# pettni/smooth_feedback

Hardware: AMD Instinct MI355X
Metric: QP solves/sec (higher is better)
Workload: dtype f64

## Files before the change

smooth_feedback_amd/csrc/qp_sparse.hip:

```cpp
#include <hip/hip_runtime.h>

#include <cstdlib>
#include <map>
#include <mutex>

#include <algorithm>
#include <type_traits>
#include <utility>
#include <cfloat>
#include <cmath>

#include "knobs.h"
#include "../../include/sfb.h"
#include "qp_sparse_kernel.h"
#include "wave_util.h"

#ifndef SFB_SWEEP_ASM
#define SFB_SWEEP_ASM 1
#endif
#ifndef SFB_SWEEP_DEPTH
#define SFB_SWEEP_DEPTH 8
#endif

namespace sfb {

namespace {

__device__ __forceinline__ int uni(const int v) { return __builtin_amdgcn_readfirstlane(v); }

struct Ws {
  double *Lx, *LxF, *LxB, *D, *Dinv, *tv;
  double *sx, *qc, *xs, *xus, *dxus;
  double *sy, *rho, *rinv, *lo, *hi, *ys, *zs, *yus, *zus, *dyus, *act;
  double *hdr;
  double *Axc;
};
constexpr int kHdrStamp = 6, kHdrC = 7, kHdrSigma = 8, kHdrScaling = 9;
constexpr int kHdrCode = 10, kHdrComplete = 11;
[[maybe_unused]] constexpr int kHdrTl2 = 12;
enum { PH_SETUP = 1, PH_ADMM = 2, PH_FINISH = 3 };
constexpr int phases_pack(int ph0, int ph1, unsigned pause_at = 0, int dq_mode = 0)
{
  return ph0 | (ph1 << 4) | (int)((pause_at & 0xFFFFFu) << 8) | (dq_mode << 28);
}
constexpr int PH_EVERYTHING = phases_pack(PH_SETUP, PH_FINISH);
constexpr unsigned long long kFactorStamp = 0x5FB0FAC7A11CE5EDull;

__device__ __forceinline__ Ws carve_ws(double *base, int n, int m, int nnzL, int funits, int bunits)
{
  const int k = n + m;
  Ws w;
  double *p = base;
  w.Lx = p; p += nnzL;
  w.D = p; p += k;
  p += 2;
  w.LxF = p; p += (size_t)(funits + kSweepPadDev) * 128;
  w.LxB = p; p += (size_t)(bunits + kSweepPadDev) * 128;
  w.Dinv = p; p += k;   w.tv = p; p += k;
  w.sx = p; p += n;     w.qc = p; p += n;     w.xs = p; p += n;   w.xus = p; p += n;  w.dxus = p; p += n;
  p += n;
  w.sy = p; p += m;     w.rho = p; p += m;    w.rinv = p; p += m; w.lo = p; p += m;   w.hi = p; p += m;
  w.ys = p; p += m;     w.zs = p; p += m;     w.yus = p; p += m;  w.zus = p; p += m;  w.dyus = p; p += m;
  w.act = p; p += m;
  w.hdr = p; p += 16;
  w.Axc = p;
  return w;
}
__device__ __forceinline__ Ws polish_ws(const Ws &w, double *base, const size_t off, int n, int m, int nnzL, int funits, int bunits)
{
  const int k = n + m;
  Ws v = w;
  double *p = base + off;
  v.Lx = p; p += nnzL;
  v.D = p; p += k;
  p += 2;
  v.LxF = p; p += (size_t)(funits + kSweepPadDev) * 128;
  v.LxB = p; p += (size_t)(bunits + kSweepPadDev) * 128;
  v.Dinv = p;
// ... 847 lines not shown
__device__ inline void ldl_solve_dev(const SparsePlanDev &pl, const Ws &w, double *t, const int lane, const bool lean,
                                     const double *dinv_lds = nullptr)
{
  const double *const Dinv = dinv_lds ? dinv_lds : w.Dinv;
  const int k = uni(pl.k);
  const bool bo = uni(pl.idx_scale) == 8;
  auto sweep = [&](const int32_t *idx, const int units, const double *vals, const int32_t *mask, const int f0, const int f1) {
    if (lean) {
      vdouble2 lx[SFB_SWEEP_DEPTH];
      vint2 ix[SFB_SWEEP_DEPTH];
      if (bo) sweep_dev<SFB_SWEEP_DEPTH, true, true>(idx, units, vals, t, lane, mask, f0, f1, lx, ix);
      else sweep_dev<SFB_SWEEP_DEPTH, false, true>(idx, units, vals, t, lane, mask, f0, f1, lx, ix);
    } else {
      vdouble2 lx[SD];
      vint2 ix[SD];
      if (bo) sweep_dev<SD, true, false>(idx, units, vals, t, lane, mask, f0, f1, lx, ix);
      else sweep_dev<SD, false, false>(idx, units, vals, t, lane, mask, f0, f1, lx, ix);
    }
  };
  sweep(pl.fidx, uni(pl.funits), w.LxF, pl.fmask, uni(pl.ffull0), uni(pl.ffull1));
  for (int j0 = lane; j0 < k; j0 += kWave * 8) {
    double dv[8];
#pragma unroll
    for (int e = 0; e < 8; ++e) dv[e] = (j0 + e * kWave < k) ? Dinv[j0 + e * kWave] : 0.0;
#pragma unroll
    for (int e = 0; e < 8; ++e)
      if (j0 + e * kWave < k) t[j0 + e * kWave] = dv[e] * t[j0 + e * kWave];
  }
  wave_sync();
  sweep(pl.bidx, uni(pl.bunits), w.LxB, pl.bmask, uni(pl.bfull0), uni(pl.bfull1));
}

constexpr int kLatRegRows = 12;
__host__ __device__ constexpr size_t lat_lds_doubles(const int n, const int m)
{
  const size_t lay = (size_t)(((n + m + 2) + 1) & ~1) + n + 2 * (size_t)m + (n + m) + 8 + (2 * kLatRegRows * 64) / 4 + (kLatRegRows * 64) / 8 + 4;
  const size_t rows = (size_t)(((n + m + 2) + 1) & ~1) + kLatRegRows * 64;
  return lay > rows ? lay : rows;
}
#ifndef SFB_LAT_TAIL
#define SFB_LAT_TAIL 48
#endif
constexpr int kLatTail = SFB_LAT_TAIL;
constexpr int kLatTailMax = 48;
static_assert(kLatTail >= 0 && kLatTail <= kLatTailMax && kLatTail % 8 == 0, "the forward sweep ends on a block of 8 units; lanes 0 .. kLatTail");
constexpr int kLatTailReg0 = 256 - 2 * kLatTail;
constexpr int kLatResident = ((kLatTailReg0 - kAgprFree) / 4) & ~7;
__device__ __forceinline__ int lat_tail_units(const SparsePlanDev &pl)
{
  const int ft = uni(pl.ftail);
  return (kLatTail > 0 && uni(pl.idx_scale) == 8 && uni(pl.ftail0) >= 8) ? (ft < kLatTail ? ft : kLatTail) : 0;
}
__device__ __forceinline__ bool lat_resident_ok(const SparsePlanDev &pl, const int treg) { return uni(pl.funits) - treg >= kLatResident + 16; }
__device__ __forceinline__ void lat_resident_load(const double *LxF, const int lane)
{
  asm volatile("" ::: "a255");
  const vdouble2 *p = reinterpret_cast<const vdouble2 *>(LxF) + lane;
  auto for_units = [&]<int... U>(std::integer_sequence<int, U...>, auto &&fn) { (fn(std::integral_constant<int, U>{}), ...); };
  for_units(std::make_integer_sequence<int, kLatResident / 4>{}, [&]<int G>(std::integral_constant<int, G>) {
    const vdouble2 *pg = p + G * 4 * kWave;
    asm volatile("global_load_dwordx4 a[%1:%2], %0, off\n\t"
                 "global_load_dwordx4 a[%3:%4], %0, off offset:1024\n\t"
                 "global_load_dwordx4 a[%5:%6], %0, off offset:2048\n\t"
                 "global_load_dwordx4 a[%7:%8], %0, off offset:3072"
                 :
                 : "v"(pg), "n"(kAgprFree + 16 * G), "n"(kAgprFree + 16 * G + 3), "n"(kAgprFree + 16 * G + 4), "n"(kAgprFree + 16 * G + 7),
                   "n"(kAgprFree + 16 * G + 8), "n"(kAgprFree + 16 * G + 11), "n"(kAgprFree + 16 * G + 12), "n"(kAgprFree + 16 * G + 15)
                 : "memory");
  });
  asm volatile("s_waitcnt vmcnt(0)" ::: "memory");
}
__device__ __forceinline__ unsigned long long lat_tail_load(const SparsePlanDev &pl, const double *LxF, const int lane, const int treg)
{
  asm volatile("" ::: "a255");
  unsigned long long have = 0;
  const int i0 = uni(pl.ftail) - kLatTail;
  const int32_t *pos = pl.ftpos + (lane + i0);
  auto for_steps = [&]<int... S>(std::integer_sequence<int, S...>, auto &&fn) { (fn(std::integral_constant<int, S>{}), ...); };
  for_steps(std::make_integer_sequence<int, kLatTail>{}, [&]<int S>(std::integral_constant<int, S>) {
    const bool on = S >= kLatTail - treg && lane > S && lane <= kLatTail;
    const int q   = on ? pos[(i0 + S) * kWave] : -1;
    const double *pv = LxF + (q >= 0 ? q : 0);
    asm volatile("global_load_dwordx2 a[%1:%2], %0, off" : : "v"(pv), "n"(kLatTailReg0 + 2 * S), "n"(kLatTailReg0 + 2 * S + 1) : "memory");
    if (q >= 0) have |= 1ull << S;
  });
  asm volatile("s_waitcnt vmcnt(0)" ::: "memory");
  return have;
}
__device__ __forceinline__ void ldl_solve_lat(const SparsePlanDev &pl, const Ws &w, double *t, const int lane, const double *Dinv,
                                              vdouble2 (&lx)[8], vint2 (&ix)[8], const bool pre, const bool next, const bool resident = false,
                                              const int treg = 0, const unsigned long long tail_have = 0)
{
  const int k = uni(pl.k);
  const int fu = uni(pl.funits) - treg;
  if (resident) sweep_dev<8, true, false, false, true, kLatResident>(pl.fidx, fu, w.LxF, t, lane, pl.fmask, 0, 0, lx, ix, pl.bidx, w.LxB, pl.bmask);
  else if (pre) sweep_dev<8, true, false, true, true>(pl.fidx, fu, w.LxF, t, lane, pl.fmask, 0, 0, lx, ix, pl.bidx, w.LxB, pl.bmask);
  else sweep_dev<8, true, false, false, true>(pl.fidx, fu, w.LxF, t, lane, pl.fmask, 0, 0, lx, ix, pl.bidx, w.LxB, pl.bmask);
  if constexpr (kLatTail > 0) {
    if (treg > 0) {
      double *const tl = t + (k - 1 - kLatTail) + lane;
      const bool mine = lane >= kLatTail - treg && lane <= kLatTail;
      double tr = mine ? *tl : 0.0;
      auto for_steps = [&]<int... S>(std::integer_sequence<int, S...>, auto &&fn) { (fn(std::integral_constant<int, S>{}), ...); };
      auto block = [&]<int B>(std::integral_constant<int, B>) {
        if (8 * B + 8 > kLatTail - treg) {
          for_steps(std::make_integer_sequence<int, 8>{}, [&]<int E>(std::integral_constant<int, E>) {
            constexpr int S = 8 * B + E;
            int l0, h0;
            asm volatile("v_accvgpr_read_b32 %0, a[%2] ; lat tail (check_sweep_spills.py)\n\tv_accvgpr_read_b32 %1, a[%3]"
                         : "=v"(l0), "=v"(h0)
                         : "n"(kLatTailReg0 + 2 * S), "n"(kLatTailReg0 + 2 * S + 1));
            const double piv = __hiloint2double(__builtin_amdgcn_readlane(__double2hiint(tr), S), __builtin_amdgcn_readlane(__double2loint(tr), S));
            if ((tail_have >> S) & 1) tr = fma(-__hiloint2double(h0, l0), piv, tr);
          });
        }
      };
      for_steps(std::make_integer_sequence<int, kLatTail / 8>{}, block);
      if (mine && lane > kLatTail - treg) *tl = tr;
      wave_lds_fence();
    }
  }
  for (int j0 = lane; j0 < k; j0 += kWave * 8) {
    double dv[8];
#pragma unroll
    for (int e = 0; e < 8; ++e) dv[e] = (j0 + e * kWave < k) ? Dinv[j0 + e * kWave] : 0.0;
#pragma unroll
    for (int e = 0; e < 8; ++e)
      if (j0 + e * kWave < k) t[j0 + e * kWave] = dv[e] * t[j0 + e * kWave];
  }
  wave_lds_fence();
  if (next) sweep_dev<8, true, false, true, true>(pl.bidx, uni(pl.bunits), w.LxB, t, lane, pl.bmask, 0, 0, lx, ix, pl.fidx, w.LxF, pl.fmask);
  else sweep_dev<8, true, false, true, false>(pl.bidx, uni(pl.bunits), w.LxB, t, lane, pl.bmask, 0, 0, lx, ix);
}

template<int UB>
__device__ __forceinline__ double lane_max_abs_b(const double *v, const int len, const int lane)
{
  double r = 0.0;
  for (int e0 = lane; e0 < len; e0 += kWave * UB) {
    double x[UB];
#pragma unroll
    for (int e = 0; e < UB; ++e) x[e] = (e0 + e * kWave < len) ? v[e0 + e * kWave] : 0.0;
#pragma unroll
    for (int e = 0; e < UB; ++e) r = fmax(r, fabs(x[e]));
  }
  return wave_max(r);
}
__device__ __forceinline__ double lane_max_abs(const double *v, int len, int lane)
{
  double r = 0.0;
// ... 691 lines not shown
      for (int e = 0; e < UB; ++e)
        if (p0 + e * kWave < nnzA) w.Axc[p0 + e * kWave] = v[e];
    }
    it.Ax = w.Axc;
    wave_sync();
  }

  bool keep_scaling = keep && !kp.scaling;
  if (kp.scaling) {
    for (int j = lane; j < n; j += kWave) {
      double v = 0.0;
      for (int p = pl.Pp[j]; p < pl.Pp[j + 1]; ++p) v = fmax(v, fabs(it.Px[p]));
      if (v == 0.0) v = 1.0;
      t[j] = v;
    }
    wave_sync();
    double sum = t[0];
    {
      int j = 1;
      for (; j + 16 <= n; j += 16) {
        double v[16];
#pragma unroll
        for (int qq = 0; qq < 16; ++qq) v[qq] = t[j + qq];
#pragma unroll
        for (int qq = 0; qq < 16; ++qq) sum += v[qq];
      }
      for (; j < n; ++j) sum += t[j];
    }
    const double qn = lane_max_abs(it.q, n, lane);
    c               = 1.0 / fmax(fmax(1e-6, sum / (double)n), qn);
    wave_sync();
    keep_scaling = keep && c == w.hdr[kHdrC];
  }
  if (!keep_scaling) {
    for (int j = lane; j < n; j += kWave) w.sx[j] = 1.0;
    for (int i = lane; i < m; i += kWave) w.sy[i] = 1.0;
    wave_sync();
  }
  if (kp.scaling && !keep_scaling) {
    int pass = 0;
    double crit;
    do {
      for (int e = lane; e < k; e += kWave) t[e] = 0.0;
      wave_sync();
      constexpr int UB = 8;
      {
        int rr[UB], cc[UB];
        double pv[UB];
        auto fetchP = [&](const int p0) {
#pragma unroll
          for (int e = 0; e < UB; ++e) {
            const int p = p0 + e * kWave;
            const bool on = p < nnzP;
            rr[e] = on ? pl.Pi[p] : 0;
            cc[e] = on ? pl.Pcol[p] : 0;
            pv[e] = on ? it.Px[p] : 0.0;
          }
        };
        fetchP(lane);
        for (int p0 = lane; p0 < nnzP; p0 += kWave * UB) {
          int c0[UB];
          double v0[UB], sr[UB], sc[UB];
#pragma unroll
          for (int e = 0; e < UB; ++e) {
            sr[e] = w.sx[rr[e]];
            sc[e] = w.sx[cc[e]];
            c0[e] = cc[e];
            v0[e] = pv[e];
          }
          fetchP(p0 + kWave * UB);
#pragma unroll
          for (int e = 0; e < UB; ++e)
// ... 26 lines not shown
            c0[e] = cc[e];
            v0[e] = av[e];
          }
          fetchA(p0 + kWave * UB);
#pragma unroll
          for (int e = 0; e < UB; ++e) {
            if (p0 + e * kWave < nnzA) {
              const double v = fabs(sr[e] * sc[e] * v0[e]);
              __hip_atomic_fetch_max(&t[c0[e]], v, __ATOMIC_RELAXED, __HIP_MEMORY_SCOPE_WORKGROUP);
              __hip_atomic_fetch_max(&t[n + r0[e]], v, __ATOMIC_RELAXED, __HIP_MEMORY_SCOPE_WORKGROUP);
            }
          }
        }
      }
      wave_sync();
      double cm = 0.0;
      for (int e = lane; e < k; e += kWave) {
        double inc = t[e];
        if (inc == 0.0) inc = 1.0;
        t[e] = inc;
        cm   = fmax(cm, fabs(inc - 1.0));
      }
      wave_sync();
      for (int j = lane; j < n; j += kWave) w.sx[j] = sqrt(1.0 / fmax(t[j], 1e-8)) * w.sx[j];
      for (int i = lane; i < m; i += kWave) w.sy[i] = sqrt(1.0 / fmax(t[n + i], 1e-8)) * w.sy[i];
      crit = wave_max(cm);
      wave_sync();
    } while (pass++ < 10 && crit > 0.1);
  }

  bool keep_factor = keep_scaling;
  {
    bool bad = false, rho_changed = false;
    for (int i = lane; i < m; i += kWave) {
      const double li = it.l[i], ui = it.u[i], syi = w.sy[i];
      bad = bad || (li == inf) || (ui == -inf) || (ui - li < 0.0);
      double rho;
      if (li == -inf && ui == inf) rho = 1e-6;
      else if (syi * fabs(li - ui) < 1e-5) rho = 1e3 * kp.rho_bar;
      else rho = kp.rho_bar;
      if (keep_scaling) rho_changed = rho_changed || !(w.rho[i] == rho);
      w.rho[i]  = rho;
      w.rinv[i] = 1.0 / rho;
      w.lo[i]   = syi * li;
      w.hi[i]   = syi * ui;
    }
    for (int j = lane; j < n; j += kWave) w.qc[j] = c * w.sx[j] * it.q[j];
    if (wave_ballot(bad)) ret_code = SFB_QP_PRIMAL_INFEASIBLE;
    if (keep_scaling && wave_ballot(rho_changed)) keep_factor = false;
  }
  wave_sync();

  phase_lap(0);
  if (!keep_factor) {
    if (lane == 0) w.hdr[kHdrStamp] = 0.0;
    if (!ldl_numeric_dev<8>(pl, it, w, t, 0, c, kp.sigma, kp.delta, lane, TRACE ? &ph_fill : nullptr)) {
      ret_code = SFB_QP_UNKNOWN;
    } else if (lane == 0 && allow_reuse) {
      w.hdr[kHdrStamp]   = __longlong_as_double((long long)kFactorStamp);
      w.hdr[kHdrC]       = c;
      w.hdr[kHdrSigma]   = kp.sigma;
      w.hdr[kHdrScaling] = (double)kp.scaling;
    }
  }

  if constexpr (TRACE) {
    phase_lap(2);
    ph_t[1] = ph_fill;
    ph_t[2] -= ph_fill;
  }
#ifdef SFB_SP_TIMELINE
  tl1 = wall_clock64();
#endif
  if (gwx != nullptr) {
    const double *wx = gwx + b * (size_t)n, *wy = gwy + b * (size_t)m;
    for (int j = lane; j < n; j += kWave) w.xs[j] = (1.0 / w.sx[j]) * wx[j];
    for (int i = lane; i < m; i += kWave) {
      const double syi = w.sy[i];
      w.ys[i]          = c * ((1.0 / syi) * wy[i]);
      double acc       = 0.0;
// ... 704 lines not shown
      }
    }
    item   = __builtin_amdgcn_readfirstlane(item);
    resume = __builtin_amdgcn_readfirstlane(resume);
    const int lean_waves_item = lean_waves;
    if (item < 0) break;
    if (resume) __builtin_amdgcn_fence(__ATOMIC_ACQUIRE, "agent");
    const bool helper = LAT && resume == 2;
    if (dq_mode == 2 || helper) resume = 0;
    wave_sync();
    const SparsePlanDev *use = plp;
    double *wsb              = gws;
    size_t wsd = ws_doubles, slot = (queue == nullptr) ? (size_t)blockIdx.x : (size_t)item;
    int fbslot = -1;
    if (plf != nullptr && !resume && ph0 <= PH_SETUP && !sp_guard_ok(*plp, gAx + (size_t)item * (size_t)uni(plp->nnzA_io), lane)) {
      if (lane == 0) {
        for (int probe = blockIdx.x % nfb;; probe = (probe + 1) % nfb) {
          if (atomicCAS(&fbflags[probe], 0, 1) == 0) { fbslot = probe; break; }
          __builtin_amdgcn_s_sleep(8);
        }
      }
      fbslot = __builtin_amdgcn_readfirstlane(fbslot);
      use = plf; wsb = gwsf; wsd = wsf_doubles; slot = (size_t)fbslot;
    }
    int seen = 0;
    const bool counts_own = dq_mode == 2 || (LAT && ((phases >> 28) & 1) == 1);
    if (counts_own && lane == 0) atomicAdd(&(fbflags + kFbSlots + 2 * batch + 16)[kDqOwn], 1);
    int32_t *const active = plp->dev_active;
    if (lane == 0) seen = atomicAdd(active, 1);
    const bool lean = (nwaves > lean_waves_item) || __builtin_amdgcn_readfirstlane(seen) >= lean_waves_item;
    const int st = sp_solve_item<LAT, TRACE, LAT || POLISHER>(*use, kp, gPx, gq, gAx, gl, gu, gwx, gwy, gx, gy, gobj, giter, gcode, wsb, wsd, lean_waves_item,
                                 lean, (size_t)item, slot, t, lane, resume != 0, fbslot >= 0 ? nullptr : queue, nfresh, slice,
                                  fbslot < 0 && slot == (size_t)item,
                                 fbslot >= 0 ? PH_EVERYTHING : (helper ? (PH_FINISH | (PH_FINISH << 4)) : phases), keys ? keys + item : nullptr, trace,
                                 trace_cap, phase_us);
    if (keys != nullptr && st != SP_PAUSED && lane == 0) keys[item] = -1.0f;
    if (fbslot >= 0 && phases != PH_EVERYTHING && lane == 0)
      carve_ws(gws + (size_t)item * ws_doubles, uni(plp->n), uni(plp->m), uni(plp->nnzL), uni(plp->funits), uni(plp->bunits)).hdr[kHdrComplete] = 1.0;
    if ((dq_mode == 2 || helper) && lane == 0)
      carve_ws(gws + (size_t)item * ws_doubles, uni(plp->n), uni(plp->m), uni(plp->nnzL), uni(plp->funits), uni(plp->bunits)).hdr[kHdrComplete] = 1.0;
    wave_sync();
    if constexpr (LAT) {
      if (st == SP_DONE && !helper && (phases & 0xFF) == (PH_ADMM | (PH_ADMM << 4)) && ((phases >> 28) & 1) == 1 && lane == 0) {
        int32_t *const doneq = fbflags + kFbSlots + 2 * batch + 16;
        __builtin_amdgcn_fence(__ATOMIC_RELEASE, "agent");
        asm volatile("s_waitcnt vmcnt(0)" ::: "memory");
        const int tl = atomicAdd(&doneq[kDqTail], 1);
        __hip_atomic_store(&doneq[kDqRing + tl], item + 1, __ATOMIC_RELAXED, __HIP_MEMORY_SCOPE_AGENT);
      }
    }
    if (lane == 0) {
      atomicSub(active, 1);
      if (counts_own) atomicSub(&(fbflags + kFbSlots + 2 * batch + 16)[kDqOwn], 1);
      if (fbslot >= 0) __hip_atomic_store(&fbflags[fbslot], 0, __ATOMIC_RELEASE, __HIP_MEMORY_SCOPE_AGENT);
      if (st == SP_SUSPENDED) {
        __builtin_amdgcn_fence(__ATOMIC_RELEASE, "agent");
        asm volatile("s_waitcnt vmcnt(0)" ::: "memory");
        const int tl = atomicAdd(&queue[kQTail], 1);
        int32_t *e   = &queue[kQRing + (unsigned)tl % (unsigned)batch];
        while (__hip_atomic_load(e, __ATOMIC_RELAXED, __HIP_MEMORY_SCOPE_AGENT) != 0) __builtin_amdgcn_s_sleep(4);
        __hip_atomic_store(e, item + 1, __ATOMIC_RELAXED, __HIP_MEMORY_SCOPE_AGENT);
      }
    }
    wave_sync();
    if (queue == nullptr && dq_mode != 2) break;
  }
}

__global__ void sp_gate_kernel(const int32_t *__restrict__ started)
{
// ... 234 lines not shown

hipError_t qp_sparse_launch(const SparsePlanDev &pl, const DenseKernelParams &kp, int64_t batch, const double *Px,
                            const double *q, const double *Ax, const double *l, const double *u, const double *wx,
                            const double *wy, double *x, double *y, double *obj, uint32_t *iter, int32_t *code,
                            double *workspace, hipStream_t stream, const int32_t *order, int32_t *aux,
                            const SparsePlanDev *fallback, double *fallback_ws, double *trace, int trace_cap, double *phase_us)
{
  if (pl.Aorig != nullptr && (fallback == nullptr || fallback_ws == nullptr || aux == nullptr)) return hipErrorInvalidValue;
  SparseDeviceBook *const book = sparse_book();
  if (book == nullptr) return hipErrorInvalidDevice;
  const bool pruned = pl.Aorig != nullptr;
  const size_t lds = (size_t)std::max(pl.lds_doubles, pruned ? fallback->lds_doubles : 0) * sizeof(double);
  const size_t wsd = qp_sparse_ws_doubles(pl);
  const char *lw        = sfb::knob("SFB_SP_LEAN_WAVES");
  const int lean_waves  = lw ? atoi(lw) : 512;
  const char *sl   = sfb::knob("SFB_SP_SLICE");
  const int slice  = sl ? atoi(sl) : 50;
  unsigned grid    = (unsigned)batch;
  int32_t *qarg    = nullptr;
  bool sliced      = false;
  if (aux != nullptr && slice > 0) {
    int resident = sparse_resident_blocks(*book, lds);
    if (const char *g = sfb::knob("SFB_SP_GRID"); g && atoi(g) > 0) resident = std::min(resident, atoi(g));
    const bool lat_ok  = pl.n <= kLatRegRows * kWave && pl.m <= kLatRegRows * kWave && lat_lds_doubles(pl.n, pl.m) * sizeof(double) <= 80 * 1024;
    const int64_t hold = lat_ok ? std::min<int64_t>(resident, 3 * (int64_t)book->cus) : resident;
    if (resident > 0 && batch > hold) {
      grid   = (unsigned)std::min<int64_t>(resident, batch);
      qarg   = aux;
      sliced = true;
    }
  }
  const char *ph    = sfb::knob("SFB_SP_PHASED");
  const bool phased = sliced && ph && atoi(ph) == 1;
  struct DoneQ { int32_t *q = nullptr; int mode = 0; hipStream_t on = nullptr; };
  auto launch = [&](unsigned g, int32_t *qa, int lw, int phases, const int32_t *ord = nullptr, uint32_t slc = 0, float *keys = nullptr,
                    const int32_t *nfresh = nullptr, int mode_sel = -1, bool lat = false, size_t lds_lat = 0, DoneQ dq = DoneQ{}) -> hipError_t {
    if ((qa != nullptr || pruned) && dq.mode != 2) {
      hipError_t e = hipMemsetAsync(aux, 0, sparse_aux_queue_ints(batch) * sizeof(int32_t), stream);
      if (e != hipSuccess) return e;
    }
    auto *kern = (trace || phase_us) ? qp_sparse_kernel<false, true>
                                     : (dq.mode == 2 ? qp_sparse_kernel<false, false, true> : (lat ? qp_sparse_kernel<true> : qp_sparse_kernel<false>));
    hipLaunchKernelGGL(kern, dim3(g), dim3(kWave), lat ? lds_lat : lds, dq.mode == 2 ? dq.on : stream, pl.self, kp, Px, q, Ax, l, u, wx, wy, x, y,
                       obj, iter, code, workspace, wsd, lw, ord, qa, (int)batch, slc ? slc : (uint32_t)std::max(1, slice),
                       pruned ? fallback->self : nullptr, fallback_ws, pruned ? qp_sparse_ws_doubles(*fallback) : 0,
                       aux ? aux + batch + kQRing : nullptr, phases, (int)std::min<int64_t>(batch, kFbSlots), keys, nfresh, mode_sel,
                       trace, trace_cap, phase_us);
    return hipGetLastError();
  };
  if (trace != nullptr || phase_us != nullptr) return launch((unsigned)batch, nullptr, lean_waves, PH_EVERYTHING, order);
  const char *pr       = sfb::knob("SFB_SP_PREDICT");
  const char *pa       = sfb::knob("SFB_SP_PAUSE");
  const unsigned pause = pa ? (unsigned)std::max(0, atoi(pa)) : 2u;
  const bool predicted = sliced && !phased && !(pr && atoi(pr) == 0) && pause > 0 && kp.stop_check_iter >= 2 && kp.max_iter > 2 * pause;
  if (predicted) {
    int32_t *xtra   = aux + sparse_aux_queue_ints(batch);
    float *keys     = reinterpret_cast<float *>(xtra);
    int32_t *order2 = xtra + batch, *count = xtra + 2 * batch;
    bool others_busy = false;
    const SparseDeviceBook::Slot slot = sparse_enqueue_begin(*book, stream, &others_busy);
    struct EnqueueEnd {
      SparseDeviceBook &bk;
      const SparseDeviceBook::Slot &sl;
      hipStream_t st;
      ~EnqueueEnd() { sparse_enqueue_end(bk, sl, st); }
    } enqueue_end{*book, slot, stream};
    hipError_t e = launch(grid, qarg, lean_waves, phases_pack(PH_SETUP, PH_FINISH, pause), order, 0, keys);
    if (e != hipSuccess) return e;
    const double stream_bytes = (double)(pl.funits + pl.bunits) * 128.0 * sizeof(double), mall = 256.0 * 1024.0 * 1024.0;
    unsigned g_lo = std::min(grid, ((unsigned)std::max(256.0, 0.70 * mall / stream_bytes) + 32u) / 64u * 64u), g_hi = grid;
    const size_t lds_lat = std::max(lds, lat_lds_doubles(pl.n, pl.m) * sizeof(double));
    int lat_hi = 0, lat_lo = 0;
    const bool lat_fits = lds_lat <= 80 * 1024 && pl.n <= kLatRegRows * kWave && pl.m <= kLatRegRows * kWave;
    if (const char *lt = sfb::knob("SFB_SP_LAT"); !(lt && atoi(lt) == 0) && lat_fits) {
      if (sparse_lat_opt_in(*book)) lat_hi = std::min<int>(sparse_resident_blocks(*book, lds_lat, true), (int)grid);
      if (const char *lw = sfb::knob("SFB_SP_LAT_WAVES"); lw && atoi(lw) > 0) lat_hi = std::min(lat_hi, atoi(lw));
      lat_lo = std::min(lat_hi, 448);
    }
    const int lat_max = 0x7FFFFFFF;
// ... 85 lines not shown
```

smooth_feedback_amd/csrc/knobs.cpp:

```cpp
#include "knobs.h"

#include <atomic>
#include <cstdio>
#include <cstring>
#include <deque>
#include <map>
#include <mutex>
#include <string>

namespace sfb {

namespace {
const char *const kKnobs[] = {"SFB_SP_GRID",  "SFB_SP_SLICE",  "SFB_SP_PAUSE",      "SFB_SP_PREDICT",   "SFB_SP_LAT",
                              "SFB_SP_FORCE_LAT", "SFB_SP_LAT_WAVES", "SFB_SP_POLISHERS", "SFB_SP_LAT_HELP", "SFB_SP_PHASED", "SFB_SP_LEAN_WAVES", "SFB_MID_GRID", "SFB_MID_SLICE",
                              "SFB_QP4_MAX_WAVES", "SFB_QP_DENSE_BIG", "SFB_EKF_PERSISTENT", "SFB_PLAN_UNITS", "SFB_PLAN_DEBUG", "SFB_MPC_TIMING", "SFB_NLP_AGENTS",
                              "SFB_NLP_HESS_AGENTS"};
std::mutex g_mu;
std::atomic<int> g_set{0};
std::map<std::string, const char *> &table()
{
  static std::map<std::string, const char *> t;
  return t;
}
const char *intern(const char *value)
{
  static std::deque<std::string> pool;
  for (const auto &v : pool)
    if (v == value) return v.c_str();
  pool.emplace_back(value);
  return pool.back().c_str();
}
}

const char *knob(const char *name)
{
  if (g_set.load(std::memory_order_acquire) == 0) return nullptr;
  std::lock_guard<std::mutex> lk(g_mu);
  const auto &t = table();
  const auto it = t.find(name);
  return it == t.end() ? nullptr : it->second;
}

int knob_set(const char *name, const char *value)
{
  if (name == nullptr) return 1;
  bool known = false;
  for (const char *k : kKnobs) known = known || std::strcmp(k, name) == 0;
// ... 16 lines not shown
```

Measured before the change: 233,200.

## Run LDL forward-solve tail with DPP row-broadcast FMA chain in inline asm

Replaces the serial per-step readlane-and-FMA loop over the last 48 units of the forward triangular sweep with a hand-written inline-asm sequence. It uses v_fmac_f64_dpp row_newbcast to broadcast each pivot within a 16-lane row, plus per-step exec masks built from ballot-derived lane sets. The tail load now stores per-lane step masks and loads -0.0 for diagonal lanes. The aim is to shorten the cross-lane latency chain in the tail, but it adds a non-finite check with a fallback to the old readlane path, hard-codes SGPR/VGPR numbers, and carries correctness risk.

Result: no change. 234,500 (median of 6 runs) (+0.6%).

```diff
diff --git a/smooth_feedback_amd/csrc/qp_sparse.hip b/smooth_feedback_amd/csrc/qp_sparse.hip
--- a/smooth_feedback_amd/csrc/qp_sparse.hip
+++ b/smooth_feedback_amd/csrc/qp_sparse.hip
@@ -970,6 +970,11 @@
 constexpr int kLatTailMax = 48;
 static_assert(kLatTail >= 0 && kLatTail <= kLatTailMax && kLatTail % 8 == 0, "the forward sweep ends on a block of 8 units; lanes 0 .. kLatTail");
 constexpr int kLatTailReg0 = 256 - 2 * kLatTail;
+#ifndef SFB_LAT_TAIL_DPP
+#define SFB_LAT_TAIL_DPP 1
+#endif
+constexpr bool kLatTailDpp = SFB_LAT_TAIL_DPP != 0 && kLatTail == 48;
+__device__ const double kLatNegZero = -0.0;
 constexpr int kLatResident = ((kLatTailReg0 - kAgprFree) / 4) & ~7;
 __device__ __forceinline__ int lat_tail_units(const SparsePlanDev &pl)
 {
@@ -1006,12 +1011,113 @@
     const bool on = S >= kLatTail - treg && lane > S && lane <= kLatTail;
     const int q   = on ? pos[(i0 + S) * kWave] : -1;
     const double *pv = LxF + (q >= 0 ? q : 0);
+    if constexpr (kLatTailDpp) pv = lane == S ? &kLatNegZero : pv;
     asm volatile("global_load_dwordx2 a[%1:%2], %0, off" : : "v"(pv), "n"(kLatTailReg0 + 2 * S), "n"(kLatTailReg0 + 2 * S + 1) : "memory");
-    if (q >= 0) have |= 1ull << S;
+    if constexpr (kLatTailDpp) {
+      const unsigned long long lanes = wave_ballot(q >= 0) | (1ull << S);
+      have = lane == S ? lanes : have;
+    } else {
+      if (q >= 0) have |= 1ull << S;
+    }
   });
   asm volatile("s_waitcnt vmcnt(0)" ::: "memory");
   return have;
 }
+#if SFB_LAT_TAIL_DPP
+#define SFB_LT_X64E "s_mov_b64 exec, s[92:93] ; lat tail (check_sweep_spills.py)\n\t"
+#define SFB_LT_X64O "s_mov_b64 exec, s[94:95] ; lat tail (check_sweep_spills.py)\n\t"
+#define SFB_LT_X32E "s_mov_b32 exec_hi, s93 ; lat tail (check_sweep_spills.py)\n\t"
+#define SFB_LT_X32O "s_mov_b32 exec_hi, s95 ; lat tail (check_sweep_spills.py)\n\t"
+#define SFB_LT_F64E(S) "v_readlane_b32 s92, %[slo], " #S "\n\tv_readlane_b32 s93, %[shi], " #S "\n\t"
+#define SFB_LT_F64O(S) "v_readlane_b32 s94, %[slo], " #S "\n\tv_readlane_b32 s95, %[shi], " #S "\n\t"
+#define SFB_LT_F32E(S) "v_readlane_b32 s93, %[shi], " #S "\n\t"
+#define SFB_LT_F32O(S) "v_readlane_b32 s95, %[shi], " #S "\n\t"
+#define SFB_LT_PIVOT(S) "v_readlane_b32 vcc_lo, v254, " #S "\n\tv_readlane_b32 vcc_hi, v255, " #S "\n\t"
+#define SFB_LT_OPND(LO, HI) "v_accvgpr_read_b32 v252, a[" #LO "]\n\tv_accvgpr_read_b32 v253, a[" #HI "]\n\t"
+#define SFB_LT_CHAIN(J, RM) "v_fmac_f64_dpp v[254:255], v[254:255], -v[252:253] row_newbcast:" #J " row_mask:" #RM " bank_mask:0xf\n\t"
+#define SFB_LT_BEHIND "v_fma_f64 %[b], -v[252:253], vcc, %[b]\n\t"
+#define SFB_LT_ROWS(LO, HI) "s_mov_b32 exec_lo, " #LO " ; lat tail (check_sweep_spills.py)\n\ts_mov_b32 exec_hi, " #HI "\n\tv_mov_b64 v[254:255], %[b]\n\t"
+#define SFB_LT_HEAD0
+#define SFB_LT_HEAD1
+#define SFB_LT_HEAD2 SFB_LT_ROWS(0xffff0000, 0x1ffff)
+#define SFB_LT_HEAD3
+#define SFB_LT_HEAD4 SFB_LT_ROWS(0, 0x1ffff)
+#define SFB_LT_HEAD5 "s_mov_b32 exec_lo, 0\n\t"
+#define SFB_LT_ENTER(T, HB) "s_cmp_lt_i32 %[treg], " #T "\n\ts_cbranch_scc0 .Lin" #HB "_%=\n\t"
+#define SFB_LT_IN(HB, S) ".Lin" #HB "_%=:\n\t" SFB_LT_F64E(S) "s_branch .Llt" #HB "_%=\n\t"
+__device__ __forceinline__ void lat_tail_dpp(double &tr, const unsigned long long step_lanes, const int treg)
+{
+  static_assert(!kLatTailDpp || kLatTailReg0 == 160, "the AccVGPR numbers below");
+  const int slo = (int)(unsigned)step_lanes, shi = (int)(unsigned)(step_lanes >> 32);
+  double b;
+  asm volatile(
+    "v_mov_b64 v[254:255], %[tr] ; lat tail (check_sweep_spills.py)\n\t"
+    "v_mov_b64 %[b], %[tr]\n\t"
+    SFB_LT_ENTER(48, 0) SFB_LT_ENTER(40, 1) SFB_LT_ENTER(32, 2) SFB_LT_ENTER(24, 3) SFB_LT_ENTER(16, 4)
+    SFB_LT_IN(5, 40) SFB_LT_IN(4, 32) SFB_LT_IN(3, 24) SFB_LT_IN(2, 16) SFB_LT_IN(1, 8)
+    ".Lin0_%=:\n\t" SFB_LT_F64E(0)
+    ".Llt0_%=:\n\t" SFB_LT_HEAD0
+    SFB_LT_X64E SFB_LT_PIVOT(0) SFB_LT_F64O(1) SFB_LT_OPND(160, 161) SFB_LT_CHAIN(0, 1) SFB_LT_BEHIND
+    SFB_LT_X64O SFB_LT_PIVOT(1) SFB_LT_F64E(2) SFB_LT_OPND(162, 163) SFB_LT_CHAIN(1, 1) SFB_LT_BEHIND
+    SFB_LT_X64E SFB_LT_PIVOT(2) SFB_LT_F64O(3) SFB_LT_OPND(164, 165) SFB_LT_CHAIN(2, 1) SFB_LT_BEHIND
+    SFB_LT_X64O SFB_LT_PIVOT(3) SFB_LT_F64E(4) SFB_LT_OPND(166, 167) SFB_LT_CHAIN(3, 1) SFB_LT_BEHIND
+    SFB_LT_X64E SFB_LT_PIVOT(4) SFB_LT_F64O(5) SFB_LT_OPND(168, 169) SFB_LT_CHAIN(4, 1) SFB_LT_BEHIND
+    SFB_LT_X64O SFB_LT_PIVOT(5) SFB_LT_F64E(6) SFB_LT_OPND(170, 171) SFB_LT_CHAIN(5, 1) SFB_LT_BEHIND
+    SFB_LT_X64E SFB_LT_PIVOT(6) SFB_LT_F64O(7) SFB_LT_OPND(172, 173) SFB_LT_CHAIN(6, 1) SFB_LT_BEHIND
+    SFB_LT_X64O SFB_LT_PIVOT(7) SFB_LT_F64E(8) SFB_LT_OPND(174, 175) SFB_LT_CHAIN(7, 1) SFB_LT_BEHIND
+    ".Llt1_%=:\n\t" SFB_LT_HEAD1
+    SFB_LT_X64E SFB_LT_PIVOT(8) SFB_LT_F64O(9) SFB_LT_OPND(176, 177) SFB_LT_CHAIN(8, 1) SFB_LT_BEHIND
+    SFB_LT_X64O SFB_LT_PIVOT(9) SFB_LT_F64E(10) SFB_LT_OPND(178, 179) SFB_LT_CHAIN(9, 1) SFB_LT_BEHIND
+    SFB_LT_X64E SFB_LT_PIVOT(10) SFB_LT_F64O(11) SFB_LT_OPND(180, 181) SFB_LT_CHAIN(10, 1) SFB_LT_BEHIND
+    SFB_LT_X64O SFB_LT_PIVOT(11) SFB_LT_F64E(12) SFB_LT_OPND(182, 183) SFB_LT_CHAIN(11, 1) SFB_LT_BEHIND
+    SFB_LT_X64E SFB_LT_PIVOT(12) SFB_LT_F64O(13) SFB_LT_OPND(184, 185) SFB_LT_CHAIN(12, 1) SFB_LT_BEHIND
+    SFB_LT_X64O SFB_LT_PIVOT(13) SFB_LT_F64E(14) SFB_LT_OPND(186, 187) SFB_LT_CHAIN(13, 1) SFB_LT_BEHIND
+    SFB_LT_X64E SFB_LT_PIVOT(14) SFB_LT_F64O(15) SFB_LT_OPND(188, 189) SFB_LT_CHAIN(14, 1) SFB_LT_BEHIND
+    SFB_LT_X64O SFB_LT_PIVOT(15) SFB_LT_F64E(16) SFB_LT_OPND(190, 191) SFB_LT_BEHIND
+    ".Llt2_%=:\n\t" SFB_LT_HEAD2
+    SFB_LT_X64E SFB_LT_PIVOT(16) SFB_LT_F64O(17) SFB_LT_OPND(192, 193) SFB_LT_CHAIN(0, 2) SFB_LT_BEHIND
+    SFB_LT_X64O SFB_LT_PIVOT(17) SFB_LT_F64E(18) SFB_LT_OPND(194, 195) SFB_LT_CHAIN(1, 2) SFB_LT_BEHIND
+    SFB_LT_X64E SFB_LT_PIVOT(18) SFB_LT_F64O(19) SFB_LT_OPND(196, 197) SFB_LT_CHAIN(2, 2) SFB_LT_BEHIND
+    SFB_LT_X64O SFB_LT_PIVOT(19) SFB_LT_F64E(20) SFB_LT_OPND(198, 199) SFB_LT_CHAIN(3, 2) SFB_LT_BEHIND
+    SFB_LT_X64E SFB_LT_PIVOT(20) SFB_LT_F64O(21) SFB_LT_OPND(200, 201) SFB_LT_CHAIN(4, 2) SFB_LT_BEHIND
+    SFB_LT_X64O SFB_LT_PIVOT(21) SFB_LT_F64E(22) SFB_LT_OPND(202, 203) SFB_LT_CHAIN(5, 2) SFB_LT_BEHIND
+    SFB_LT_X64E SFB_LT_PIVOT(22) SFB_LT_F64O(23) SFB_LT_OPND(204, 205) SFB_LT_CHAIN(6, 2) SFB_LT_BEHIND
+    SFB_LT_X64O SFB_LT_PIVOT(23) SFB_LT_F64E(24) SFB_LT_OPND(206, 207) SFB_LT_CHAIN(7, 2) SFB_LT_BEHIND
+    ".Llt3_%=:\n\t" SFB_LT_HEAD3
+    SFB_LT_X64E SFB_LT_PIVOT(24) SFB_LT_F64O(25) SFB_LT_OPND(208, 209) SFB_LT_CHAIN(8, 2) SFB_LT_BEHIND
+    SFB_LT_X64O SFB_LT_PIVOT(25) SFB_LT_F64E(26) SFB_LT_OPND(210, 211) SFB_LT_CHAIN(9, 2) SFB_LT_BEHIND
+    SFB_LT_X64E SFB_LT_PIVOT(26) SFB_LT_F64O(27) SFB_LT_OPND(212, 213) SFB_LT_CHAIN(10, 2) SFB_LT_BEHIND
+    SFB_LT_X64O SFB_LT_PIVOT(27) SFB_LT_F64E(28) SFB_LT_OPND(214, 215) SFB_LT_CHAIN(11, 2) SFB_LT_BEHIND
+    SFB_LT_X64E SFB_LT_PIVOT(28) SFB_LT_F64O(29) SFB_LT_OPND(216, 217) SFB_LT_CHAIN(12, 2) SFB_LT_BEHIND
+    SFB_LT_X64O SFB_LT_PIVOT(29) SFB_LT_F64E(30) SFB_LT_OPND(218, 219) SFB_LT_CHAIN(13, 2) SFB_LT_BEHIND
+    SFB_LT_X64E SFB_LT_PIVOT(30) SFB_LT_F64O(31) SFB_LT_OPND(220, 221) SFB_LT_CHAIN(14, 2) SFB_LT_BEHIND
+    SFB_LT_X64O SFB_LT_PIVOT(31) SFB_LT_F32E(32) SFB_LT_OPND(222, 223) SFB_LT_BEHIND
+    ".Llt4_%=:\n\t" SFB_LT_HEAD4
+    SFB_LT_X32E SFB_LT_PIVOT(32) SFB_LT_F32O(33) SFB_LT_OPND(224, 225) SFB_LT_CHAIN(0, 4) SFB_LT_BEHIND
+    SFB_LT_X32O SFB_LT_PIVOT(33) SFB_LT_F32E(34) SFB_LT_OPND(226, 227) SFB_LT_CHAIN(1, 4) SFB_LT_BEHIND
+    SFB_LT_X32E SFB_LT_PIVOT(34) SFB_LT_F32O(35) SFB_LT_OPND(228, 229) SFB_LT_CHAIN(2, 4) SFB_LT_BEHIND
+    SFB_LT_X32O SFB_LT_PIVOT(35) SFB_LT_F32E(36) SFB_LT_OPND(230, 231) SFB_LT_CHAIN(3, 4) SFB_LT_BEHIND
+    SFB_LT_X32E SFB_LT_PIVOT(36) SFB_LT_F32O(37) SFB_LT_OPND(232, 233) SFB_LT_CHAIN(4, 4) SFB_LT_BEHIND
+    SFB_LT_X32O SFB_LT_PIVOT(37) SFB_LT_F32E(38) SFB_LT_OPND(234, 235) SFB_LT_CHAIN(5, 4) SFB_LT_BEHIND
+    SFB_LT_X32E SFB_LT_PIVOT(38) SFB_LT_F32O(39) SFB_LT_OPND(236, 237) SFB_LT_CHAIN(6, 4) SFB_LT_BEHIND
+    SFB_LT_X32O SFB_LT_PIVOT(39) SFB_LT_F32E(40) SFB_LT_OPND(238, 239) SFB_LT_CHAIN(7, 4) SFB_LT_BEHIND
+    ".Llt5_%=:\n\t" SFB_LT_HEAD5
+    SFB_LT_X32E SFB_LT_PIVOT(40) SFB_LT_F32O(41) SFB_LT_OPND(240, 241) SFB_LT_CHAIN(8, 4) SFB_LT_BEHIND
+    SFB_LT_X32O SFB_LT_PIVOT(41) SFB_LT_F32E(42) SFB_LT_OPND(242, 243) SFB_LT_CHAIN(9, 4) SFB_LT_BEHIND
+    SFB_LT_X32E SFB_LT_PIVOT(42) SFB_LT_F32O(43) SFB_LT_OPND(244, 245) SFB_LT_CHAIN(10, 4) SFB_LT_BEHIND
+    SFB_LT_X32O SFB_LT_PIVOT(43) SFB_LT_F32E(44) SFB_LT_OPND(246, 247) SFB_LT_CHAIN(11, 4) SFB_LT_BEHIND
+    SFB_LT_X32E SFB_LT_PIVOT(44) SFB_LT_F32O(45) SFB_LT_OPND(248, 249) SFB_LT_CHAIN(12, 4) SFB_LT_BEHIND
+    SFB_LT_X32O SFB_LT_PIVOT(45) SFB_LT_F32E(46) SFB_LT_OPND(250, 251) SFB_LT_CHAIN(13, 4) SFB_LT_BEHIND
+    SFB_LT_X32E SFB_LT_PIVOT(46) SFB_LT_F32O(47) SFB_LT_OPND(252, 253) SFB_LT_CHAIN(14, 4) SFB_LT_BEHIND
+    SFB_LT_X32O SFB_LT_PIVOT(47) SFB_LT_OPND(254, 255) SFB_LT_BEHIND
+    SFB_LT_ROWS(0, 0x10000)
+    "s_mov_b64 exec, -1\n\t"
+    "v_mov_b64 %[tr], v[254:255]"
+    : [tr] "+v"(tr), [b] "=&v"(b)
+    : [slo] "v"(slo), [shi] "v"(shi), [treg] "s"(treg)
+    : "v252", "v253", "v254", "v255", "s92", "s93", "s94", "s95", "vcc", "scc");
+}
+#endif
 __device__ __forceinline__ void ldl_solve_lat(const SparsePlanDev &pl, const Ws &w, double *t, const int lane, const double *Dinv,
                                               vdouble2 (&lx)[8], vint2 (&ix)[8], const bool pre, const bool next, const bool resident = false,
                                               const int treg = 0, const unsigned long long tail_have = 0)
@@ -1027,20 +1133,39 @@
       const bool mine = lane >= kLatTail - treg && lane <= kLatTail;
       double tr = mine ? *tl : 0.0;
       auto for_steps = [&]<int... S>(std::integer_sequence<int, S...>, auto &&fn) { (fn(std::integral_constant<int, S>{}), ...); };
-      auto block = [&]<int B>(std::integral_constant<int, B>) {
-        if (8 * B + 8 > kLatTail - treg) {
-          for_steps(std::make_integer_sequence<int, 8>{}, [&]<int E>(std::integral_constant<int, E>) {
-            constexpr int S = 8 * B + E;
-            int l0, h0;
-            asm volatile("v_accvgpr_read_b32 %0, a[%2] ; lat tail (check_sweep_spills.py)\n\tv_accvgpr_read_b32 %1, a[%3]"
-                         : "=v"(l0), "=v"(h0)
-                         : "n"(kLatTailReg0 + 2 * S), "n"(kLatTailReg0 + 2 * S + 1));
-            const double piv = __hiloint2double(__builtin_amdgcn_readlane(__double2hiint(tr), S), __builtin_amdgcn_readlane(__double2loint(tr), S));
-            if ((tail_have >> S) & 1) tr = fma(-__hiloint2double(h0, l0), piv, tr);
+      auto readlane_steps = [&](const unsigned long long have) {
+        auto block = [&]<int B>(std::integral_constant<int, B>) {
+          if (8 * B + 8 > kLatTail - treg) {
+            for_steps(std::make_integer_sequence<int, 8>{}, [&]<int E>(std::integral_constant<int, E>) {
+              constexpr int S = 8 * B + E;
+              int l0, h0;
+              asm volatile("v_accvgpr_read_b32 %0, a[%2] ; lat tail (check_sweep_spills.py)\n\tv_accvgpr_read_b32 %1, a[%3]"
+                           : "=v"(l0), "=v"(h0)
+                           : "n"(kLatTailReg0 + 2 * S), "n"(kLatTailReg0 + 2 * S + 1));
+              const double piv = __hiloint2double(__builtin_amdgcn_readlane(__double2hiint(tr), S), __builtin_amdgcn_readlane(__double2loint(tr), S));
+              if ((have >> S) & 1) tr = fma(-__hiloint2double(h0, l0), piv, tr);
+            });
+          }
+        };
+        for_steps(std::make_integer_sequence<int, kLatTail / 8>{}, block);
+      };
+#if SFB_LAT_TAIL_DPP
+      if constexpr (kLatTailDpp) {
+        lat_tail_dpp(tr, tail_have, treg);
+        if (wave_ballot(mine && !(fabs(tr) <= DBL_MAX))) {
+          tr = mine ? *tl : 0.0;
+          unsigned long long have = 0;
+          for_steps(std::make_integer_sequence<int, kLatTail>{}, [&]<int S>(std::integral_constant<int, S>) {
+            const unsigned lo = (unsigned)__builtin_amdgcn_readlane((int)(unsigned)tail_have, S);
+            const unsigned hi = (unsigned)__builtin_amdgcn_readlane((int)(unsigned)(tail_have >> 32), S);
+            const unsigned long long lanes = ((unsigned long long)hi << 32) | lo;
+            if (lane > S && ((lanes >> lane) & 1)) have |= 1ull << S;
           });
-        }
-      };
-      for_steps(std::make_integer_sequence<int, kLatTail / 8>{}, block);
+          readlane_steps(have);
+        }
+      } else
+#endif
+      readlane_steps(tail_have);
       if (mine && lane > kLatTail - treg) *tl = tr;
       wave_lds_fence();
     }
```

## Run Ruiz equilibration on-chip with row scales in registers and column scales in LDS

Applied to the files above, without the earlier changes.

Replaces the global-memory Ruiz scaling loop in the sparse QP setup with an on-chip variant. Row scale factors live in per-lane registers, and column scales plus column maxima live in LDS, updated with workgroup-scope atomic max. Global sx/sy are written only once at the end. This is meant to cut repeated global workspace traffic and barriers during setup. The cost is added register pressure, plus an old-path opt-out knob whose flag bit is threaded through the phases word.

New measurement: 233,600 before, 234,400 after (median of 6 runs). No clear change (+0.4%).

```diff
diff --git a/smooth_feedback_amd/csrc/knobs.cpp b/smooth_feedback_amd/csrc/knobs.cpp
--- a/smooth_feedback_amd/csrc/knobs.cpp
+++ b/smooth_feedback_amd/csrc/knobs.cpp
@@ -12,7 +12,7 @@
 
 namespace {
 const char *const kKnobs[] = {"SFB_SP_GRID",  "SFB_SP_SLICE",  "SFB_SP_PAUSE",      "SFB_SP_PREDICT",   "SFB_SP_LAT",
-                              "SFB_SP_FORCE_LAT", "SFB_SP_LAT_WAVES", "SFB_SP_POLISHERS", "SFB_SP_LAT_HELP", "SFB_SP_PHASED", "SFB_SP_LEAN_WAVES", "SFB_MID_GRID", "SFB_MID_SLICE",
+                              "SFB_SP_FORCE_LAT", "SFB_SP_LAT_WAVES", "SFB_SP_POLISHERS", "SFB_SP_LAT_HELP", "SFB_SP_PHASED", "SFB_SP_LEAN_WAVES", "SFB_SP_SETUP_OLD", "SFB_MID_GRID", "SFB_MID_SLICE",
                               "SFB_QP4_MAX_WAVES", "SFB_QP_DENSE_BIG", "SFB_EKF_PERSISTENT", "SFB_PLAN_UNITS", "SFB_PLAN_DEBUG", "SFB_MPC_TIMING", "SFB_NLP_AGENTS",
                               "SFB_NLP_HESS_AGENTS"};
 std::mutex g_mu;
diff --git a/smooth_feedback_amd/csrc/qp_sparse.hip b/smooth_feedback_amd/csrc/qp_sparse.hip
--- a/smooth_feedback_amd/csrc/qp_sparse.hip
+++ b/smooth_feedback_amd/csrc/qp_sparse.hip
@@ -44,6 +44,7 @@
   return ph0 | (ph1 << 4) | (int)((pause_at & 0xFFFFFu) << 8) | (dq_mode << 28);
 }
 constexpr int PH_EVERYTHING = phases_pack(PH_SETUP, PH_FINISH);
+constexpr int kSetupOldBits = 1 << 30;
 constexpr unsigned long long kFactorStamp = 0x5FB0FAC7A11CE5EDull;
 
 __device__ __forceinline__ Ws carve_ws(double *base, int n, int m, int nnzL, int funits, int bunits)
@@ -957,6 +958,7 @@
 }
 
 constexpr int kLatRegRows = 12;
+constexpr int kRuizRows   = kLatRegRows;
 __host__ __device__ constexpr size_t lat_lds_doubles(const int n, const int m)
 {
   const size_t lay = (size_t)(((n + m + 2) + 1) & ~1) + n + 2 * (size_t)m + (n + m) + 8 + (2 * kLatRegRows * 64) / 4 + (kLatRegRows * 64) / 8 + 4;
@@ -1798,12 +1800,134 @@
     wave_sync();
     keep_scaling = keep && c == w.hdr[kHdrC];
   }
-  if (!keep_scaling) {
+  const bool ruiz_on_chip = !LAT && kp.scaling && !keep_scaling && ((phases >> 30) & 1) == 0 && 2 * n <= uni(pl.lds_doubles) && m <= kRuizRows * kWave;
+  double sy_reg[kRuizRows];
+  if (!keep_scaling && !ruiz_on_chip) {
     for (int j = lane; j < n; j += kWave) w.sx[j] = 1.0;
     for (int i = lane; i < m; i += kWave) w.sy[i] = 1.0;
     wave_sync();
   }
-  if (kp.scaling && !keep_scaling) {
+  if (ruiz_on_chip) {
+    constexpr int RS = 2, CE = 4, UB = 4;
+    int rp0[kRuizRows];
+#pragma unroll
+    for (int r = 0; r < kRuizRows; ++r) {
+      const int i = lane + r * kWave;
+      rp0[r]    = pl.Ap[i < m ? i : m];
+      sy_reg[r] = 1.0;
+    }
+    const int rp_end = uni(pl.Ap[m]);
+    auto row_end = [&](const int r) {
+      const int nxt  = __shfl_down(rp0[r], 1);
+      const int wrap = r + 1 < kRuizRows ? __builtin_amdgcn_readlane(rp0[r + 1 < kRuizRows ? r + 1 : r], 0) : rp_end;
+      return lane == kWave - 1 ? wrap : nxt;
+    };
+    for (int j = lane; j < n; j += kWave) {
+      t[j]     = 1.0;
+      t[n + j] = 0.0;
+    }
+    wave_lds_fence();
+    int pass = 0;
+    double crit;
+    do {
+      double cm = 0.0;
+      {
+        int rr[UB], cc[UB];
+        double pv[UB];
+        auto fetchP = [&](const int p0) {
+#pragma unroll
+          for (int e = 0; e < UB; ++e) {
+            const int p = p0 + e * kWave;
+            const bool on = p < nnzP;
+            rr[e] = on ? pl.Pi[p] : 0;
+            cc[e] = on ? pl.Pcol[p] : 0;
+            pv[e] = on ? it.Px[p] : 0.0;
+          }
+        };
+        fetchP(lane);
+        for (int p0 = lane; p0 < nnzP; p0 += kWave * UB) {
+          int r0[UB], c0[UB];
+          double v0[UB];
+#pragma unroll
+          for (int e = 0; e < UB; ++e) {
+            r0[e] = rr[e];
+            c0[e] = cc[e];
+            v0[e] = pv[e];
+          }
+          fetchP(p0 + kWave * UB);
+#pragma unroll
+          for (int e = 0; e < UB; ++e)
+            if (p0 + e * kWave < nnzP)
+              __hip_atomic_fetch_max(&t[n + c0[e]], fabs(c * t[r0[e]] * t[c0[e]] * v0[e]), __ATOMIC_RELAXED, __HIP_MEMORY_SCOPE_WORKGROUP);
+        }
+      }
+#pragma unroll
+      for (int s = 0; s < kRuizRows; s += RS) {
+        if (s * kWave < m) {
+          int q[RS], q1[RS];
+          double rinc[RS];
+#pragma unroll
+          for (int r = 0; r < RS; ++r) {
+            q[r]    = rp0[s + r];
+            q1[r]   = row_end(s + r);
+            rinc[r] = 0.0;
+          }
+          bool more;
+          do {
+            int cj[RS][CE];
+            double av[RS][CE];
+#pragma unroll
+            for (int r = 0; r < RS; ++r) {
+#pragma unroll
+              for (int e = 0; e < CE; ++e) {
+                const bool on = q[r] + e < q1[r];
+                cj[r][e] = on ? pl.Aj[q[r] + e] : 0;
+                av[r][e] = on ? it.Ax[q[r] + e] : 0.0;
+              }
+            }
+            more = false;
+#pragma unroll
+            for (int r = 0; r < RS; ++r) {
+#pragma unroll
+              for (int e = 0; e < CE; ++e) {
+                if (q[r] + e < q1[r]) {
+                  const double v = fabs(sy_reg[s + r] * t[cj[r][e]] * av[r][e]);
+                  rinc[r] = fmax(rinc[r], v);
+                  __hip_atomic_fetch_max(&t[n + cj[r][e]], v, __ATOMIC_RELAXED, __HIP_MEMORY_SCOPE_WORKGROUP);
+                }
+              }
+              __builtin_amdgcn_sched_barrier(0);
+              q[r] += CE;
+              more = more || q[r] < q1[r];
+            }
+          } while (wave_ballot(more));
+#pragma unroll
+          for (int r = 0; r < RS; ++r) {
+            if (lane + (s + r) * kWave < m) {
+              double inc = rinc[r];
+              if (inc == 0.0) inc = 1.0;
+              cm            = fmax(cm, fabs(inc - 1.0));
+              sy_reg[s + r] = sqrt(1.0 / fmax(inc, 1e-8)) * sy_reg[s + r];
+            }
+          }
+        }
+      }
+      wave_lds_fence();
+      for (int j = lane; j < n; j += kWave) {
+        double inc = t[n + j];
+        if (inc == 0.0) inc = 1.0;
+        cm       = fmax(cm, fabs(inc - 1.0));
+        t[j]     = sqrt(1.0 / fmax(inc, 1e-8)) * t[j];
+        t[n + j] = 0.0;
+      }
+      wave_lds_fence();
+      crit = wave_max(cm);
+    } while (pass++ < 10 && crit > 0.1);
+    for (int j = lane; j < n; j += kWave) w.sx[j] = t[j];
+#pragma unroll
+    for (int r = 0; r < kRuizRows; ++r)
+      if (lane + r * kWave < m) w.sy[lane + r * kWave] = sy_reg[r];
+  } else if (kp.scaling && !keep_scaling) {
     int pass = 0;
     double crit;
     do {
@@ -1896,8 +2020,8 @@
   bool keep_factor = keep_scaling;
   {
     bool bad = false, rho_changed = false;
-    for (int i = lane; i < m; i += kWave) {
-      const double li = it.l[i], ui = it.u[i], syi = w.sy[i];
+    auto row = [&](const int i, const double syi) {
+      const double li = it.l[i], ui = it.u[i];
       bad = bad || (li == inf) || (ui == -inf) || (ui - li < 0.0);
       double rho;
       if (li == -inf && ui == inf) rho = 1e-6;
@@ -1908,8 +2032,18 @@
       w.rinv[i] = 1.0 / rho;
       w.lo[i]   = syi * li;
       w.hi[i]   = syi * ui;
-    }
-    for (int j = lane; j < n; j += kWave) w.qc[j] = c * w.sx[j] * it.q[j];
+    };
+    if (ruiz_on_chip) {
+#pragma unroll
+      for (int r = 0; r < kRuizRows; ++r)
+        if (lane + r * kWave < m) row(lane + r * kWave, sy_reg[r]);
+      for (int j = lane; j < n; j += kWave) w.qc[j] = c * t[j] * it.q[j];
+      wave_lds_fence();
+      if (lane == 0) t[k] = 0.0;
+    } else {
+      for (int i = lane; i < m; i += kWave) row(i, w.sy[i]);
+      for (int j = lane; j < n; j += kWave) w.qc[j] = c * w.sx[j] * it.q[j];
+    }
     if (wave_ballot(bad)) ret_code = SFB_QP_PRIMAL_INFEASIBLE;
     if (keep_scaling && wave_ballot(rho_changed)) keep_factor = false;
   }
@@ -2680,10 +2814,10 @@
     const int st = sp_solve_item<LAT, TRACE, LAT || POLISHER>(*use, kp, gPx, gq, gAx, gl, gu, gwx, gwy, gx, gy, gobj, giter, gcode, wsb, wsd, lean_waves_item,
                                  lean, (size_t)item, slot, t, lane, resume != 0, fbslot >= 0 ? nullptr : queue, nfresh, slice,
                                   fbslot < 0 && slot == (size_t)item,
-                                 fbslot >= 0 ? PH_EVERYTHING : (helper ? (PH_FINISH | (PH_FINISH << 4)) : phases), keys ? keys + item : nullptr, trace,
+                                 fbslot >= 0 ? (PH_EVERYTHING | (phases & kSetupOldBits)) : (helper ? (PH_FINISH | (PH_FINISH << 4) | (phases & kSetupOldBits)) : phases), keys ? keys + item : nullptr, trace,
                                  trace_cap, phase_us);
     if (keys != nullptr && st != SP_PAUSED && lane == 0) keys[item] = -1.0f;
-    if (fbslot >= 0 && phases != PH_EVERYTHING && lane == 0)
+    if (fbslot >= 0 && (phases & ~kSetupOldBits) != PH_EVERYTHING && lane == 0)
       carve_ws(gws + (size_t)item * ws_doubles, uni(plp->n), uni(plp->m), uni(plp->nnzL), uni(plp->funits), uni(plp->bunits)).hdr[kHdrComplete] = 1.0;
     if ((dq_mode == 2 || helper) && lane == 0)
       carve_ws(gws + (size_t)item * ws_doubles, uni(plp->n), uni(plp->m), uni(plp->nnzL), uni(plp->funits), uni(plp->bunits)).hdr[kHdrComplete] = 1.0;
@@ -2984,6 +3118,8 @@
   }
   const char *ph    = sfb::knob("SFB_SP_PHASED");
   const bool phased = sliced && ph && atoi(ph) == 1;
+  const char *so      = sfb::knob("SFB_SP_SETUP_OLD");
+  const int setup_old = (so && atoi(so) == 1) ? kSetupOldBits : 0;
   struct DoneQ { int32_t *q = nullptr; int mode = 0; hipStream_t on = nullptr; };
   auto launch = [&](unsigned g, int32_t *qa, int lw, int phases, const int32_t *ord = nullptr, uint32_t slc = 0, float *keys = nullptr,
                     const int32_t *nfresh = nullptr, int mode_sel = -1, bool lat = false, size_t lds_lat = 0, DoneQ dq = DoneQ{}) -> hipError_t {
@@ -2996,7 +3132,7 @@
     hipLaunchKernelGGL(kern, dim3(g), dim3(kWave), lat ? lds_lat : lds, dq.mode == 2 ? dq.on : stream, pl.self, kp, Px, q, Ax, l, u, wx, wy, x, y,
                        obj, iter, code, workspace, wsd, lw, ord, qa, (int)batch, slc ? slc : (uint32_t)std::max(1, slice),
                        pruned ? fallback->self : nullptr, fallback_ws, pruned ? qp_sparse_ws_doubles(*fallback) : 0,
-                       aux ? aux + batch + kQRing : nullptr, phases, (int)std::min<int64_t>(batch, kFbSlots), keys, nfresh, mode_sel,
+                       aux ? aux + batch + kQRing : nullptr, phases | setup_old, (int)std::min<int64_t>(batch, kFbSlots), keys, nfresh, mode_sel,
                        trace, trace_cap, phase_us);
     return hipGetLastError();
   };
```
